# splinterhq/libsplinter

Hardware: AMD Instinct MI355X
Metric: KV set/get ops/sec + Nomic-768d embed vectors/sec at 1/2/4/8 MI355X (higher is better)
Workload: dtype bf16

## Files before the change

libsplinter_amd/csrc/hip/gemm_bf16.hip:

```cpp
#include <hip/hip_runtime.h>
#include <cstdint>
#include <cstdlib>
#include <map>
#include <mutex>
#include <type_traits>

#include "glds_asm.hpp"
#include "nomic_api.h"

namespace {

typedef __bf16 bf16x8 __attribute__((ext_vector_type(8)));
typedef float f32x4 __attribute__((ext_vector_type(4)));
typedef __attribute__((address_space(3))) void lds_void;
typedef const __attribute__((address_space(1))) void gbl_void;

constexpr int BM = 128, BN = 128, BK = 64;
constexpr int kThreads = 256;
constexpr int kTileBytes = BM * BK * 2;
constexpr int kEpiStride = BN + 4;
constexpr int kLdsBytes = (BM * kEpiStride * 4 > 4 * kTileBytes) ? BM * kEpiStride * 4 : 4 * kTileBytes;

__device__ __forceinline__ float bf2f(uint16_t h) { return __uint_as_float((uint32_t)h << 16); }
typedef __bf16 bf16x2_t __attribute__((ext_vector_type(2)));
// ... 39 lines not shown
  const uint16_t* res;
  long ldr;
  const float* rope;
  const int32_t* pos;
  int rope_cols;
  long M;
  int gn;
  const float2* pin;
  int np;
  float eps;
  const float* c1;
  const float* c2;
  const uint16_t* lng;
  const uint16_t* lnb;
  float2* part;
};

constexpr bool is_fold(int m) { return m == NOMIC_EPI_ROPE_FOLD || m == NOMIC_EPI_SWIGLU_FOLD; }
constexpr bool is_stats(int m) { return m == NOMIC_EPI_RES_STATS || m == NOMIC_EPI_RES_LN_STATS; }
constexpr bool is_rope(int m) { return m == NOMIC_EPI_ROPE || m == NOMIC_EPI_ROPE_FOLD; }
constexpr bool is_swiglu(int m) { return m == NOMIC_EPI_SWIGLU || m == NOMIC_EPI_SWIGLU_FOLD; }
constexpr bool is_rowstore(int m) { return m == NOMIC_EPI_STORE || m == NOMIC_EPI_RESIDUAL || is_stats(m); }
constexpr bool needs_rowstats(int m) { return is_fold(m) || m == NOMIC_EPI_RES_LN_STATS; }

__device__ __forceinline__ float fold(float acc, float2 st, float c1, float c2) {
  return st.y * (acc - st.x * c1) + c2;
}

template <int CTRL>
__device__ __forceinline__ float dpp_add(float v) {
// ... 256 lines not shown
    for (int it = 0; it < (BM * BN / 4) / kThreads; ++it) {
      const int q = tid + it * kThreads;
      const int row = q >> 5, c4 = (q & 31) * 4;
      const long gm = m0 + row;
      if (gm >= ep.M) continue;
      *(float4*)(outf + gm * ep.ldo + n0 + c4) = *(const float4*)&E[row * kEpiStride + c4];
    }
  }
}

constexpr int kThreads2 = 512;
constexpr int kHalfBytes = 128 * BK * 2;
constexpr int kBufBytes = 4 * kHalfBytes;
constexpr int kEpi2Stride = 256 + 4;
constexpr int kLds2Bytes = (128 * kEpi2Stride * 4 > 2 * kBufBytes) ? 128 * kEpi2Stride * 4 : 2 * kBufBytes;

__device__ __forceinline__ void wait_vm(int n) {
  switch (n) {
    case 26: asm volatile("s_waitcnt vmcnt(26)" ::: "memory"); break;
    case 20: asm volatile("s_waitcnt vmcnt(20)" ::: "memory"); break;
    case 18: asm volatile("s_waitcnt vmcnt(18)" ::: "memory"); break;
    case 10: asm volatile("s_waitcnt vmcnt(10)" ::: "memory"); break;
    case 8: asm volatile("s_waitcnt vmcnt(8)" ::: "memory"); break;
    case 6: asm volatile("s_waitcnt vmcnt(6)" ::: "memory"); break;
    case 4: asm volatile("s_waitcnt vmcnt(4)" ::: "memory"); break;
    case 2: asm volatile("s_waitcnt vmcnt(2)" ::: "memory"); break;
    default: asm volatile("s_waitcnt vmcnt(0)" ::: "memory"); break;
  }
}

// ... 8 lines not shown
  o.x = pk2(v[0], v[1]);
  o.y = pk2(v[2], v[3]);
  o.z = pk2(v[4], v[5]);
  o.w = pk2(v[6], v[7]);
  return o;
}

template <int MODE, int ILV = 0, int EPI = 0, int PP = 0>
__global__ __launch_bounds__(kThreads2, 1) void k_gemm256(const uint16_t* __restrict__ A, long lda,
                                                          const uint16_t* __restrict__ W, long ldw, int K,
                                                          int mtiles, int ntiles, EpiArgs ep) {
  extern __shared__ __attribute__((aligned(16))) char smem[];
  const int tid = threadIdx.x, lane = tid & 63, wave = tid >> 6;
  const int wr = wave >> 2, wn = wave & 3;
  int mt, nt;
  remap_tile(blockIdx.x, mtiles * ntiles, ntiles, ep.gn, mt, nt);
  const long m0 = (long)mt * 256, n0 = (long)nt * 256;

  const int srow = lane >> 3, schunk = ((lane & 7) ^ srow) * 8;
  uint32_t offA[2][2], offB[2][2];
#pragma unroll
  for (int h = 0; h < 2; ++h)
#pragma unroll
    for (int i = 0; i < 2; ++i) {
      const int r = h * 128 + (i * 8 + wave) * 8 + srow;
      const long gr = (m0 + r < ep.M) ? m0 + r : ep.M - 1;
      offA[h][i] = (uint32_t)(gr * lda + schunk);
      offB[h][i] = (uint32_t)((n0 + r) * ldw + schunk);
    }
  auto stage_one = [&](int which, int t, int buf, int i) {
    const uint16_t* base = (which < 2 ? A : W) + (long)t * BK;
    char* dst = smem + buf * kBufBytes + which * kHalfBytes;
// ... 11 lines not shown
  const int frow = (lane & 15) * 128;
  const int fsw0 = ((0 * 4 + (lane >> 4)) ^ (lane & 7)) << 4;
  const int fsw1 = ((1 * 4 + (lane >> 4)) ^ (lane & 7)) << 4;

  f32x4 acc[2][2][4][2];
#pragma unroll
  for (int a = 0; a < 2; ++a)
#pragma unroll
    for (int b = 0; b < 2; ++b)
#pragma unroll
      for (int i = 0; i < 4; ++i)
#pragma unroll
        for (int j = 0; j < 2; ++j) acc[a][b][i][j] = f32x4{0.f, 0.f, 0.f, 0.f};

  const int nk = K / BK;
  stage(0, 0, 0); stage(2, 0, 0); stage(3, 0, 0); stage(1, 0, 0);
  if (nk > 1) { stage(0, 1, 1); stage(2, 1, 1); stage(3, 1, 1); }

  bf16x8 af[4][2], b0[2][2], b1[2][2];
  auto mma_phase = [&](f32x4 (&ac)[4][2], bf16x8 (&bf)[2][2], int which, int st, int sbuf, bool go) {
    if (ILV == 0 && go) stage(which, st, sbuf);
    __builtin_amdgcn_s_setprio(1);
#pragma unroll
    for (int kk = 0; kk < 2; ++kk)
#pragma unroll
      for (int i = 0; i < 4; ++i) {
        if constexpr (ILV > 0) {
          if (go && kk * 4 + i == ILV) stage_one(which, st, sbuf, 0);
          if (go && kk * 4 + i == ILV + 4) stage_one(which, st, sbuf, 1);
        }
#pragma unroll
        for (int j = 0; j < 2; ++j)
          ac[i][j] = __builtin_amdgcn_mfma_f32_16x16x32_bf16(af[i][kk], bf[j][kk], ac[i][j], 0, 0, 0);
        if constexpr (ILV > 0) __builtin_amdgcn_sched_barrier(0);
// ... 186 lines not shown
    for (int j = 0; j < 2; ++j) {
      b1[j][0] = *(const bf16x8*)(hB1 + (wn * 32 + j * 16) * 128 + frow + fsw0);
      b1[j][1] = *(const bf16x8*)(hB1 + (wn * 32 + j * 16) * 128 + frow + fsw1);
    }
    mma_phase(acc[0][1], b1, 0, t + 2, buf, n2);
    wait_vm(n2 ? 10 : (n1 ? 8 : 0));
    raw_barrier();
#pragma unroll
    for (int i = 0; i < 4; ++i) {
      af[i][0] = *(const bf16x8*)(hA1 + (wr * 64 + i * 16) * 128 + frow + fsw0);
      af[i][1] = *(const bf16x8*)(hA1 + (wr * 64 + i * 16) * 128 + frow + fsw1);
    }
    mma_phase(acc[1][0], b0, 2, t + 2, buf, n2);
    mma_phase(acc[1][1], b1, 3, t + 2, buf, n2);
  }
  asm volatile("s_waitcnt vmcnt(0)" ::: "memory");

  if constexpr (MODE == NOMIC_EPI_SWIGLU && EPI == 1) {
    constexpr int kS = 128 + 8;
    uint16_t* E16 = (uint16_t*)smem;
    const int fq = lane >> 4, fr = lane & 15;
    const bool odd = fr & 1;
    __syncthreads();
#pragma unroll
    for (int qm = 0; qm < 2; ++qm)
#pragma unroll
      for (int qn = 0; qn < 2; ++qn)
#pragma unroll
        for (int i = 0; i < 4; ++i) {
          uint32_t b[4];
// ... 10 lines not shown
        }
    __syncthreads();
#pragma unroll
    for (int it = 0; it < (256 * 16) / kThreads2; ++it) {
      const int q = tid + it * kThreads2;
      const int row = q >> 4, c = q & 15;
      const long gm = m0 + row;
      if (gm >= ep.M) continue;
      *(uint4*)(ep.out + gm * ep.ldo + (long)nt * 128 + c * 8) = *(const uint4*)(E16 + row * kS + c * 8);
    }
    return;
  }

  float* E = (float*)smem;
  const int fq = lane >> 4, fr = lane & 15;
#pragma unroll
  for (int qm = 0; qm < 2; ++qm) {
    __syncthreads();
#pragma unroll
    for (int qn = 0; qn < 2; ++qn)
#pragma unroll
      for (int i = 0; i < 4; ++i)
#pragma unroll
        for (int j = 0; j < 2; ++j)
#pragma unroll
          for (int r = 0; r < 4; ++r)
            E[(wr * 64 + i * 16 + fq * 4 + r) * kEpi2Stride + qn * 128 + wn * 32 + j * 16 + fr] = acc[qm][qn][i][j][r];
    __syncthreads();
    const long mh = m0 + qm * 128;
    if constexpr (MODE == NOMIC_EPI_STORE || MODE == NOMIC_EPI_RESIDUAL) {
#pragma unroll
      for (int it = 0; it < (128 * 256 / 8) / kThreads2; ++it) {
        const int q = tid + it * kThreads2;
        const int row = q >> 5, c8 = (q & 31) * 8;
        const long gm = mh + row;
        if (gm >= ep.M) continue;
        const float4 v0 = *(const float4*)&E[row * kEpi2Stride + c8];
        const float4 v1 = *(const float4*)&E[row * kEpi2Stride + c8 + 4];
        float v[8] = {v0.x, v0.y, v0.z, v0.w, v1.x, v1.y, v1.z, v1.w};
        if constexpr (MODE == NOMIC_EPI_RESIDUAL) {
          const uint4 rr = *(const uint4*)(ep.res + gm * ep.ldr + n0 + c8);
          const uint32_t rw[4] = {rr.x, rr.y, rr.z, rr.w};
#pragma unroll
          for (int e = 0; e < 4; ++e) {
// ... 55 lines not shown
      for (int it = 0; it < (128 * 256 / 4) / kThreads2; ++it) {
        const int q = tid + it * kThreads2;
        const int row = q >> 6, c4 = (q & 63) * 4;
        const long gm = mh + row;
        if (gm >= ep.M) continue;
        *(float4*)(outf + gm * ep.ldo + n0 + c4) = *(const float4*)&E[row * kEpi2Stride + c4];
      }
    }
  }
}

}

namespace {

int g_num_cus = 256;

template <typename F>
void allow_lds(F* f, int bytes) {
  (void)hipFuncSetAttribute((const void*)f, hipFuncAttributeMaxDynamicSharedMemorySize, bytes);
}

int g_variant = -1;
int gemm_variant() {
  if (g_variant < 0) {
    const char* e = getenv("NOMIC_GEMM");
    const int v = e ? atoi(e) : 0;
    g_variant = v == 128 || v == 256 ? v : 0;
  }
  return g_variant;
}
// ... 13 lines not shown
template <int MODE>
int launch(const uint16_t* A, long lda, const uint16_t* W, long ldw, long M, int N, int K, EpiArgs ep,
           hipStream_t s) {
  if (K % BK || N % BN || M <= 0) return (int)hipErrorInvalidValue;
  const long mpad = (M + 255) / 256 * 256;
  const bool fits = N % 256 == 0 && mpad * lda < (1L << 31) && (long)N * ldw < (1L << 31);
  const int var = gemm_variant();
  constexpr bool k256_ok = MODE <= NOMIC_EPI_F32;
  const long tiles256 = fits ? (mpad / 256) * (N / 256) : 0;
  static const long min_tiles = [] {
    const char* e = getenv("NOMIC_GEMM256_MIN_TILES");
    return e && atol(e) > 0 ? atol(e) : 1024L;
  }();
  if (k256_ok && fits && (var == 256 || (var == 0 && tiles256 >= min_tiles))) {
    static bool attr = [] {
      allow_lds(k_gemm256<MODE, 0, 0, 2>, kLds2Bytes);
      return true;
    }();
    (void)attr;
    const int mtiles = (int)(mpad / 256), ntiles = N / 256;
    ep.gn = band_width(ntiles, 4);
    if constexpr (k256_ok)
      hipLaunchKernelGGL((k_gemm256<MODE, 0, 0, 2>), dim3(mtiles * ntiles), dim3(kThreads2), kLds2Bytes, s, A, lda, W,
                         ldw, K, mtiles, ntiles, ep);
    return (int)hipGetLastError();
  }
  const int mtiles = (int)((M + BM - 1) / BM), ntiles = N / BN;
  ep.gn = band_width(ntiles, 8);
  constexpr int lds = kLdsBytes + (needs_rowstats(MODE) ? BM * 8 : 0);
  hipLaunchKernelGGL(k_gemm_nt<MODE>, dim3(mtiles * ntiles), dim3(kThreads), lds, s, A, lda, W, ldw, K, mtiles, ntiles,
                     ep);
  return (int)hipGetLastError();
}

}

extern "C" int nomic_gemm_set_variant(int variant) {
  const int prev = gemm_variant();
  g_variant = variant == 128 || variant == 256 ? variant : 0;
  return prev;
}

extern "C" int nomic_gemm_ln(int mode, const void* A, long lda, const void* W, long ldw, long M, int N, int K,
                             void* out, long ldo, const void* res, long ldr, const float* rope, const int32_t* pos,
                             int rope_cols, const float* part_in, int nparts, float eps, const float* c1,
                             const float* c2, const void* ln_g, const void* ln_b, float* part, hipStream_t s) {
  EpiArgs ep{(uint16_t*)out, ldo, (const uint16_t*)res, ldr, rope, pos, rope_cols, M, 1, (const float2*)part_in,
             nparts, eps, c1, c2, (const uint16_t*)ln_g, (const uint16_t*)ln_b, (float2*)part};
  if ((needs_rowstats(mode) && (!part_in || nparts < 1 || nparts > 8)) || (is_fold(mode) && (!c1 || !c2)) ||
      (is_stats(mode) && (!part || !res || N % BN)) || (mode == NOMIC_EPI_RES_LN_STATS && (!ln_g || !ln_b)) ||
      (mode == NOMIC_EPI_RESIDUAL && !res) || (is_rope(mode) && (!rope || !pos)))
    return (int)hipErrorInvalidValue;
  const auto* a = (const uint16_t*)A;
  const auto* w = (const uint16_t*)W;
  switch (mode) {
// ... 46 lines not shown
```

libsplinter_amd/csrc/hip/gemm_rln.hip:

```cpp
#include <hip/hip_runtime.h>
#include <cstdint>
#include <cstdlib>

#include "glds_asm.hpp"
#include "nomic_api.h"

namespace {

typedef __bf16 bf16x8 __attribute__((ext_vector_type(8)));
typedef __bf16 bf16x2_t __attribute__((ext_vector_type(2)));
typedef float f32x4 __attribute__((ext_vector_type(4)));
typedef __attribute__((address_space(3))) void lds_void;
typedef const __attribute__((address_space(1))) void gbl_void;

constexpr int kBM = 128;
constexpr int kN = 768;
constexpr int kBK = 32;
constexpr int kWN = kN / 4;
constexpr int kNT = kWN / 16;
constexpr int kThreads = 512;
constexpr int kRowBytes = kBK * 2;
constexpr int kABytes = kBM * kRowBytes;
constexpr int kWBytes = kN * kRowBytes;
constexpr int kGldsW = kWBytes / 1024 / 8;
constexpr int kHalfRows = 64;
constexpr int kOutRowBytes = kN * 2;
constexpr int kRowPitch = kOutRowBytes + 16;
constexpr int kHalfBytes = kHalfRows * kRowPitch;
constexpr int kEpiLds = kHalfBytes + 2 * 4 * kHalfRows * 4;

template <int PIPE> struct Pipe;
template <> struct Pipe<1> { static constexpr int NW = 2, NA = 4; };
template <> struct Pipe<2> { static constexpr int NW = 3, NA = 2; };
template <> struct Pipe<3> { static constexpr int NW = 2, NA = 2; };
template <> struct Pipe<4> { static constexpr int NW = 2, NA = 6; };
template <int PIPE>
constexpr int lds_bytes() {
  return Pipe<PIPE>::NW * kWBytes + Pipe<PIPE>::NA * kABytes > kEpiLds
             ? Pipe<PIPE>::NW * kWBytes + Pipe<PIPE>::NA * kABytes
             : kEpiLds;
}

__device__ __forceinline__ float bf2f(uint32_t h16) { return __uint_as_float(h16 << 16); }
__device__ __forceinline__ uint32_t pk2(float a, float b) {
// ... 4 lines not shown
__device__ __forceinline__ void raw_barrier() {
  asm volatile("" ::: "memory");
  __builtin_amdgcn_s_barrier();
  asm volatile("" ::: "memory");
}

__device__ __forceinline__ void wait_vm(int n) {
  switch (n) {
    case 12: asm volatile("s_waitcnt vmcnt(12)" ::: "memory"); break;
    case 6: asm volatile("s_waitcnt vmcnt(6)" ::: "memory"); break;
    case 2: asm volatile("s_waitcnt vmcnt(2)" ::: "memory"); break;
    case 1: asm volatile("s_waitcnt vmcnt(1)" ::: "memory"); break;
    default: asm volatile("s_waitcnt vmcnt(0)" ::: "memory"); break;
  }
}

__device__ __forceinline__ int swz(int r, int c) { return c ^ ((r >> 1) & 3); }

template <int PIPE, int EPI, int WM, int ILV = 0, int PF = 1, bool AS = false, bool ROT = false>
__global__ __launch_bounds__(256 * WM, 1) void k_gemm_rln(const uint16_t* __restrict__ A, long lda,
                                                          const uint16_t* __restrict__ W, long ldw, int K, long M,
                                                          const uint16_t* res, long ldr,
                                                          const uint16_t* __restrict__ gamma,
                                                          const uint16_t* __restrict__ beta, float eps,
                                                          uint16_t* out, long ldo) {
  constexpr int NW = Pipe<PIPE>::NW, NA = Pipe<PIPE>::NA;
  constexpr int LW = NW - 1, LA = NA - 1;
  constexpr int kABase = NW * kWBytes;
  constexpr int kWaves = 4 * WM, kNThreads = 64 * kWaves;
  constexpr int RW = kBM / WM, MT = RW / 16;
  constexpr int GA = 8 / kWaves, GW = 48 / kWaves;
  static_assert(EPI == 0 || WM == 2, "the LDS-staged epilogue splits the tile by wave rows");
  static_assert(EPI != 3 || MT * kNT == 48, "EPI 3 spreads 48 accumulator tiles over 24 stages");
  extern __shared__ __attribute__((aligned(16))) char smem[];
  const int tid = threadIdx.x, lane = tid & 63, wave = tid >> 6;
  const int wr = WM == 2 ? wave >> 2 : 0, wn = wave & 3;
  const long m0 = (long)blockIdx.x * kBM;

  const int drow = lane >> 2, dpc = lane & 3;
  uint32_t offA[GA];
#pragma unroll
  for (int i = 0; i < GA; ++i) {
    const int r = (wave + kWaves * i) * 16 + drow;
    const long gr = (m0 + r < M) ? m0 + r : M - 1;
    offA[i] = (uint32_t)(gr * lda + swz(r, dpc) * 8);
  }
  uint32_t offW[GW];
#pragma unroll
// ... 86 lines not shown
  auto res_load = [&](int u, uint2& d) {
    const int i = u / kNT, j = u % kNT;
    const long m = rmb + 16 * i < M ? rmb + 16 * i : M - 1;
    d = *(const uint2*)(res + m * ldr + wn * kWN + j * 16 + rcq);
  };
  auto res_add = [&](int u, const uint2& rr) {
    const int i = u / kNT, j = u % kNT;
    acc[i][j][0] += bf2f(rr.x & 0xffff);
    acc[i][j][1] += bf2f(rr.x >> 16);
    acc[i][j][2] += bf2f(rr.y & 0xffff);
    acc[i][j][3] += bf2f(rr.y >> 16);
  };
  for (int t = 0; t < nk; ++t) {
    wait_vm(younger(t));
    raw_barrier();
    if (EPI == 3 && t < 24) {
#pragma unroll
      for (int k = 0; k < 24; ++k) {
        if (t == k) {
          if (k > 0) {
            res_add(2 * (k - 1), rq[0]);
            res_add(2 * (k - 1) + 1, rq[1]);
          }
          res_load(2 * k, rq[0]);
          res_load(2 * k + 1, rq[1]);
        }
      }
    }
    if (ILV == 0) issue(t);
    const char* bw = smem + (t % NW) * kWBytes;
    const char* ba = smem + (t % NA) * kABytes;
// ... 27 lines not shown
      }
      __builtin_amdgcn_sched_barrier(0);
      w0 = x0;
      w1 = x1;
      if (PF == 2) {
        x0 = y0;
        x1 = y1;
      }
    }
    __builtin_amdgcn_s_setprio(0);
    if (ILV > 0) {
#pragma unroll
      for (int u = (kNT / 2) * ILV; u < kOps; ++u) issue_op(t, u);
    }
  }
  if constexpr (EPI == 3) {
    res_add(46, rq[0]);
    res_add(47, rq[1]);
  }
  asm volatile("s_waitcnt vmcnt(0)" ::: "memory");
  raw_barrier();

  const int rl = lane & 15, cq = (lane >> 4) * 4;
  if constexpr (EPI != 1) {
    float* red = (float*)smem;
    const long mb = m0 + wr * RW + rl;
    float s[MT] = {};
#pragma unroll
    for (int j = 0; j < kNT; ++j) {
      const int n = wn * kWN + j * 16 + cq;
#pragma unroll
      for (int i = 0; i < MT; ++i) {
        if constexpr (EPI == 0) {
          const long m = mb + 16 * i < M ? mb + 16 * i : M - 1;
          const uint2 rr = *(const uint2*)(res + m * ldr + n);
          acc[i][j][0] += bf2f(rr.x & 0xffff);
          acc[i][j][1] += bf2f(rr.x >> 16);
          acc[i][j][2] += bf2f(rr.y & 0xffff);
          acc[i][j][3] += bf2f(rr.y >> 16);
        }
        (void)n;
        s[i] += (acc[i][j][0] + acc[i][j][1]) + (acc[i][j][2] + acc[i][j][3]);
      }
    }
#pragma unroll
    for (int i = 0; i < MT; ++i) {
      s[i] += __shfl_xor(s[i], 16);
      s[i] += __shfl_xor(s[i], 32);
    }
    if (lane < 16) {
#pragma unroll
      for (int i = 0; i < MT; ++i) red[wn * kBM + wr * RW + i * 16 + rl] = s[i];
    }
    __syncthreads();
    float mean[MT];
#pragma unroll
    for (int i = 0; i < MT; ++i) {
      const int r = wr * RW + i * 16 + rl;
      mean[i] = (red[r] + red[kBM + r] + red[2 * kBM + r] + red[3 * kBM + r]) * (1.f / kN);
// ... 14 lines not shown
      s[i] += __shfl_xor(s[i], 32);
    }
    __syncthreads();
    if (lane < 16) {
#pragma unroll
      for (int i = 0; i < MT; ++i) red[wn * kBM + wr * RW + i * 16 + rl] = s[i];
    }
    __syncthreads();
    float rstd[MT];
#pragma unroll
    for (int i = 0; i < MT; ++i) {
      const int r = wr * RW + i * 16 + rl;
      const float var = (red[r] + red[kBM + r] + red[2 * kBM + r] + red[3 * kBM + r]) * (1.f / kN);
      rstd[i] = rsqrtf(var + eps);
    }
#pragma unroll
    for (int j = 0; j < kNT; ++j) {
      const int n = wn * kWN + j * 16 + cq;
      const uint2 gg = *(const uint2*)(gamma + n), bb = *(const uint2*)(beta + n);
      const float g[4] = {bf2f(gg.x & 0xffff), bf2f(gg.x >> 16), bf2f(gg.y & 0xffff), bf2f(gg.y >> 16)};
      const float be[4] = {bf2f(bb.x & 0xffff), bf2f(bb.x >> 16), bf2f(bb.y & 0xffff), bf2f(bb.y >> 16)};
#pragma unroll
      for (int i = 0; i < MT; ++i) {
        const long m = mb + 16 * i;
        float o[4];
#pragma unroll
        for (int e = 0; e < 4; ++e) o[e] = (acc[i][j][e] - mean[i]) * rstd[i] * g[e] + be[e];
        if (m < M) *(uint2*)(out + m * ldo + n) = make_uint2(pk2(o[0], o[1]), pk2(o[2], o[3]));
      }
    }
  } else {
    char* R = smem;
    float* red1 = (float*)(smem + kHalfBytes);
    float* red2 = red1 + 4 * kHalfRows;
    const int ebase = rl * kRowPitch + (wn * kWN + cq) * 2;
#pragma unroll 1
    for (int h = 0; h < 2; ++h) {
      const long mh = m0 + h * kHalfRows;
#pragma unroll 1
      for (int u = 0; u < kHalfRows / 8; ++u) {
        const int row = wave * 8 + u;
        const long gr = mh + row < M ? mh + row : M - 1;
        const uint16_t* src = res + gr * ldr + lane * 8;
        __builtin_amdgcn_global_load_lds((gbl_void*)src, (lds_void*)(R + row * kRowPitch), 16, 0, 0);
        if (lane < 32)
          __builtin_amdgcn_global_load_lds((gbl_void*)(src + 512), (lds_void*)(R + row * kRowPitch + 1024), 16, 0, 0);
      }
      asm volatile("s_waitcnt vmcnt(0)" ::: "memory");
      __syncthreads();
      const bool mine = wr == h;
      float mean[4], rstd[4];
      if (mine) {
        float sm[4] = {0.f, 0.f, 0.f, 0.f};
#pragma unroll
        for (int j = 0; j < kNT; ++j) {
#pragma unroll
          for (int i = 0; i < 4; ++i) {
            const uint2 rr = *(const uint2*)(R + ebase + i * 16 * kRowPitch + j * 32);
            acc[i][j][0] += bf2f(rr.x & 0xffff);
            acc[i][j][1] += bf2f(rr.x >> 16);
            acc[i][j][2] += bf2f(rr.y & 0xffff);
            acc[i][j][3] += bf2f(rr.y >> 16);
            sm[i] += (acc[i][j][0] + acc[i][j][1]) + (acc[i][j][2] + acc[i][j][3]);
          }
        }
#pragma unroll
        for (int i = 0; i < 4; ++i) {
          sm[i] += __shfl_xor(sm[i], 16);
          sm[i] += __shfl_xor(sm[i], 32);
          if (lane < 16) red1[wn * kHalfRows + i * 16 + rl] = sm[i];
        }
      }
      __syncthreads();
      if (mine) {
        float sq[4] = {0.f, 0.f, 0.f, 0.f};
#pragma unroll
        for (int i = 0; i < 4; ++i) {
          const int r = i * 16 + rl;
          mean[i] = (red1[r] + red1[kHalfRows + r] + red1[2 * kHalfRows + r] + red1[3 * kHalfRows + r]) * (1.f / kN);
        }
#pragma unroll
        for (int j = 0; j < kNT; ++j)
#pragma unroll
          for (int i = 0; i < 4; ++i)
#pragma unroll
            for (int e = 0; e < 4; ++e) {
              const float d = acc[i][j][e] - mean[i];
              sq[i] += d * d;
            }
#pragma unroll
        for (int i = 0; i < 4; ++i) {
          sq[i] += __shfl_xor(sq[i], 16);
          sq[i] += __shfl_xor(sq[i], 32);
          if (lane < 16) red2[wn * kHalfRows + i * 16 + rl] = sq[i];
        }
      }
      __syncthreads();
      if (mine) {
#pragma unroll
        for (int i = 0; i < 4; ++i) {
          const int r = i * 16 + rl;
          const float var = (red2[r] + red2[kHalfRows + r] + red2[2 * kHalfRows + r] + red2[3 * kHalfRows + r]) *
                            (1.f / kN);
          rstd[i] = rsqrtf(var + eps);
        }
#pragma unroll
        for (int j = 0; j < kNT; ++j) {
          const int n = wn * kWN + j * 16 + cq;
          const uint2 gg = *(const uint2*)(gamma + n), bb = *(const uint2*)(beta + n);
          const float g[4] = {bf2f(gg.x & 0xffff), bf2f(gg.x >> 16), bf2f(gg.y & 0xffff), bf2f(gg.y >> 16)};
          const float be[4] = {bf2f(bb.x & 0xffff), bf2f(bb.x >> 16), bf2f(bb.y & 0xffff), bf2f(bb.y >> 16)};
#pragma unroll
          for (int i = 0; i < 4; ++i) {
            float o[4];
#pragma unroll
            for (int e = 0; e < 4; ++e) o[e] = (acc[i][j][e] - mean[i]) * rstd[i] * g[e] + be[e];
            *(uint2*)(R + ebase + i * 16 * kRowPitch + j * 32) = make_uint2(pk2(o[0], o[1]), pk2(o[2], o[3]));
          }
        }
      }
      __syncthreads();
#pragma unroll 2
      for (int u = 0; u < kHalfRows * 96 / kThreads; ++u) {
        const int L = u * kThreads + tid;
        const int row = L / 96, pc = L - row * 96;
        const uint4 v = *(const uint4*)(R + row * kRowPitch + pc * 16);
        if (mh + row < M) *(uint4*)(out + (mh + row) * ldo + pc * 8) = v;
      }
      __syncthreads();
    }
  }
}

int g_rln_variant = -1;
int rln_pick(int v) { return v == 232 ? 232 : 222; }
int rln_variant() {
  if (g_rln_variant < 0) {
    const char* e = getenv("NOMIC_RLN");
    g_rln_variant = rln_pick(e && *e ? atoi(e) : 222);
  }
  return g_rln_variant;
}

template <int PIPE, int EPI, int WM = 2, int ILV = 0, int PF = 1, bool AS = false, bool ROT = false>
void launch_rln(unsigned blocks, hipStream_t s, const uint16_t* A, long lda, const uint16_t* W, long ldw, int K, long M,
                const uint16_t* res, long ldr, const uint16_t* gamma, const uint16_t* beta, float eps, uint16_t* out,
                long ldo) {
  static bool attr = [] {
    (void)hipFuncSetAttribute((const void*)k_gemm_rln<PIPE, EPI, WM, ILV, PF, AS, ROT>, hipFuncAttributeMaxDynamicSharedMemorySize,
                              lds_bytes<PIPE>());
    return true;
  }();
  (void)attr;
  hipLaunchKernelGGL((k_gemm_rln<PIPE, EPI, WM, ILV, PF, AS, ROT>), dim3(blocks), dim3(256 * WM), lds_bytes<PIPE>(), s, A, lda, W, ldw, K,
// ... 6 lines not shown
                                 const void* res, long ldr, const void* gamma, const void* beta, float eps, void* out,
                                 long ldo, hipStream_t s) {
  if (N != kN || K < kBK || K % kBK || M <= 0 || !A || !W || !res || !gamma || !beta || !out)
    return (int)hipErrorInvalidValue;
  if (lda % 8 || ldw % 8 || ldr % 4 || ldo % 4 || lda < K || ldw < K || ldr < N || ldo < N)
    return (int)hipErrorInvalidValue;
  if ((M - 1) * lda + K >= (1L << 32) || (long)kN * ldw >= (1L << 32)) return (int)hipErrorInvalidValue;
  static_assert(lds_bytes<2>() <= 160 * 1024, "LDS budget");
  const unsigned blocks = (unsigned)((M + kBM - 1) / kBM);
  const auto* a = (const uint16_t*)A;
  const auto* w = (const uint16_t*)W;
  const auto* r = (const uint16_t*)res;
  const auto* g = (const uint16_t*)gamma;
  const auto* b = (const uint16_t*)beta;
  auto* o = (uint16_t*)out;
  if (rln_variant() == 232 && K / kBK >= 24 && K <= 768) launch_rln<2, 3, 2, 2>(blocks, s, a, lda, w, ldw, K, M, r, ldr, g, b, eps, o, ldo);
  else launch_rln<2, 0, 2, 2>(blocks, s, a, lda, w, ldw, K, M, r, ldr, g, b, eps, o, ldo);
  return (int)hipGetLastError();
}

extern "C" int nomic_gemm_res_ln_set_variant(int variant) {
  const int prev = rln_variant();
  g_rln_variant = rln_pick(variant);
  return prev;
}
```

libsplinter_amd/csrc/include/nomic_api.h:

```cpp
#ifndef SPLINTER_NOMIC_API_H
#define SPLINTER_NOMIC_API_H
#include <stdint.h>
#include "arena_api.h"

#ifdef __cplusplus
extern "C" {
#endif

#define NOMIC_EPI_STORE    0
#define NOMIC_EPI_RESIDUAL 1
#define NOMIC_EPI_SWIGLU   2
#define NOMIC_EPI_ROPE     3
#define NOMIC_EPI_F32      4
#define NOMIC_EPI_ROPE_FOLD    5
#define NOMIC_EPI_SWIGLU_FOLD  6
#define NOMIC_EPI_RES_STATS    7
#define NOMIC_EPI_RES_LN_STATS 8

int nomic_gemm(int mode, const void *A, long lda, const void *W, long ldw, long M, int N, int K,
               void *out, long ldo, const void *res, long ldr, const float *rope, const int32_t *pos,
               int rope_cols, hipStream_t stream);
int nomic_gemm_ln(int mode, const void *A, long lda, const void *W, long ldw, long M, int N, int K, void *out,
                  long ldo, const void *res, long ldr, const float *rope, const int32_t *pos, int rope_cols,
                  const float *part_in, int nparts, float eps, const float *c1, const float *c2,
                  const void *ln_g, const void *ln_b, float *part, hipStream_t stream);
int nomic_row_stats(const float *part, int nparts, long M, float eps, float *st, hipStream_t stream);
int nomic_gemm_set_variant(int variant);

int nomic_embed_ln(const int32_t *ids, long T, const void *tok_emb, const void *type_row,
                   const void *gamma, const void *beta, float eps, void *out, hipStream_t stream);
int nomic_layernorm(const void *x, long T, const void *gamma, const void *beta, float eps, void *out,
                    hipStream_t stream);
int nomic_attention_set_variant(int variant);
int nomic_attention(const void *qkv, void *out, const int32_t *cu_seqlens, const int32_t *qblocks,
                    int nqb, int heads, float scale, hipStream_t stream);
int nomic_mean_pool(const void *x, const int32_t *cu_seqlens, int B, float *pooled, int normalize,
                    spl_arena_t arena, const int64_t *slots, const uint64_t *hashes, int32_t *status,
                    hipStream_t stream);
int nomic_dequant(int ggml_type, const void *src, long nelems, void *dst_bf16, hipStream_t stream);

#ifdef __cplusplus
}
// ... 3 lines not shown
```

libsplinter_amd/models/nomic.py:

```python
from __future__ import annotations

import ctypes
import math
import os
from dataclasses import dataclass
from typing import Dict, List, Optional, Sequence, Tuple

import numpy as np
import torch

from .. import _native as N
from ..utils.tracing import trace_range
from .gguf import DEVICE_DEQUANT, GGUFFile, GGUFWriter, dequant_host

EPI_STORE, EPI_RESIDUAL, EPI_SWIGLU, EPI_ROPE, EPI_F32 = 0, 1, 2, 3, 4
EPI_ROPE_FOLD, EPI_SWIGLU_FOLD, EPI_RES_STATS, EPI_RES_LN_STATS = 5, 6, 7, 8


@dataclass
class NomicConfig:
    vocab: int = 30528
    d: int = 768
    layers: int = 12
    heads: int = 12
# ... 24 lines not shown
        P, c_long, c_int, c_float = ctypes.c_void_p, ctypes.c_long, ctypes.c_int, ctypes.c_float
        L.nomic_gemm.argtypes = [c_int, P, c_long, P, c_long, c_long, c_int, c_int, P, c_long, P, c_long, P, P, c_int, P]
        L.nomic_gemm.restype = c_int
        L.nomic_gemm_ln.argtypes = [c_int, P, c_long, P, c_long, c_long, c_int, c_int, P, c_long, P, c_long, P, P,
                                    c_int, P, c_int, c_float, P, P, P, P, P, P]
        L.nomic_gemm_ln.restype = c_int
        L.nomic_gemm_res_ln.argtypes = [P, c_long, P, c_long, c_long, c_int, c_int, P, c_long, P, P, c_float, P,
                                        c_long, P]
        L.nomic_gemm_res_ln.restype = c_int
        L.nomic_gemm_res_ln_set_variant.argtypes = [c_int]
        L.nomic_gemm_res_ln_set_variant.restype = c_int
        L.nomic_row_stats.argtypes = [P, c_int, c_long, c_float, P, P]
        L.nomic_row_stats.restype = c_int
        L.nomic_gemm_set_variant.argtypes = [c_int]
        L.nomic_gemm_set_variant.restype = c_int
        L.nomic_attention_set_variant.argtypes = [c_int]
        L.nomic_attention_set_variant.restype = c_int
        L.nomic_embed_ln.argtypes = [P, c_long, P, P, P, P, c_float, P, P]
        L.nomic_embed_ln.restype = c_int
        L.nomic_layernorm.argtypes = [P, c_long, P, P, c_float, P, P]
        L.nomic_layernorm.restype = c_int
        L.nomic_attention.argtypes = [P, P, P, P, c_int, c_int, c_float, P]
        L.nomic_attention.restype = c_int
        L.nomic_mean_pool.argtypes = [P, P, c_int, P, c_int, N.Arena, P, P, P, P]
        L.nomic_mean_pool.restype = c_int
        L.nomic_dequant.argtypes = [c_int, P, c_long, P, P]
        L.nomic_dequant.restype = c_int
        L._nomic_declared = True
    return L

# ... 457 lines not shown
```

Baseline: 1.339 billion.

## Split tail-wave GEMM tiles into half-M blocks and add register-resident residual-LN epilogue

The 256x256 GEMM kernel now launches extra blocks for the last partial wave. Those tiles are split into two 128-row halves, each run by its own block with a three-slot pipeline, so CUs are not left idle at the tail. The CU count is now read from the device instead of being hard-coded. The residual+LayerNorm GEMM gains a new default epilogue (variant 242) that does 16-byte residual loads and stores with ds_swizzle lane exchange instead of 8-byte accesses, and the old LDS-staged epilogue is removed. The costs are extra LDS per block when splitting, a second mainloop path in the kernel, and possible tuning sensitivity.

```diff
diff --git a/libsplinter_amd/csrc/hip/gemm_bf16.hip b/libsplinter_amd/csrc/hip/gemm_bf16.hip
--- a/libsplinter_amd/csrc/hip/gemm_bf16.hip
+++ b/libsplinter_amd/csrc/hip/gemm_bf16.hip
@@ -77,6 +77,7 @@
   const uint16_t* lng;
   const uint16_t* lnb;
   float2* part;
+  int nsplit;
 };
 
 constexpr bool is_fold(int m) { return m == NOMIC_EPI_ROPE_FOLD || m == NOMIC_EPI_SWIGLU_FOLD; }
@@ -363,6 +364,8 @@
 constexpr int kBufBytes = 4 * kHalfBytes;
 constexpr int kEpi2Stride = 256 + 4;
 constexpr int kLds2Bytes = (128 * kEpi2Stride * 4 > 2 * kBufBytes) ? 128 * kEpi2Stride * 4 : 2 * kBufBytes;
+constexpr int kLds2SplitBytes = 9 * kHalfBytes;
+static_assert(kLds2SplitBytes >= kLds2Bytes && kLds2SplitBytes <= 160 * 1024, "LDS budget");
 
 __device__ __forceinline__ void wait_vm(int n) {
   switch (n) {
@@ -401,8 +404,23 @@
   const int tid = threadIdx.x, lane = tid & 63, wave = tid >> 6;
   const int wr = wave >> 2, wn = wave & 3;
   int mt, nt;
-  remap_tile(blockIdx.x, mtiles * ntiles, ntiles, ep.gn, mt, nt);
+  int bid = blockIdx.x, qh = -1;
+  {
+    const int nw = mtiles * ntiles - ep.nsplit;
+    if (bid >= nw) {
+      const int h = bid - nw, full = (ep.nsplit >> 3) << 4;
+      if (h < full) {
+        bid = nw + ((h >> 4) << 3) + (h & 7);
+        qh = (h >> 3) & 1;
+      } else {
+        bid = nw + (full >> 1) + ((h - full) >> 1);
+        qh = (h - full) & 1;
+      }
+    }
+  }
+  remap_tile(bid, mtiles * ntiles, ntiles, ep.gn, mt, nt);
   const long m0 = (long)mt * 256, n0 = (long)nt * 256;
+  if (qh >= 0 && m0 + qh * 128 >= ep.M) return;
 
   const int srow = lane >> 3, schunk = ((lane & 7) ^ srow) * 8;
   uint32_t offA[2][2], offB[2][2];
@@ -444,10 +462,88 @@
         for (int j = 0; j < 2; ++j) acc[a][b][i][j] = f32x4{0.f, 0.f, 0.f, 0.f};
 
   const int nk = K / BK;
+  bf16x8 af[4][2], b0[2][2], b1[2][2];
+  if (qh >= 0) {
+    constexpr int kStage3 = 3 * kHalfBytes;
+    const uint32_t oA[2] = {qh ? offA[1][0] : offA[0][0], qh ? offA[1][1] : offA[0][1]};
+    auto hstage = [&](int which, int t, int slot) {
+      const uint16_t* base = (which == 0 ? A : W) + (long)t * BK;
+      char* dst = smem + slot * kStage3 + which * kHalfBytes;
+#pragma unroll
+      for (int i = 0; i < 2; ++i) {
+        const uint32_t off = which == 0 ? oA[i] : which == 1 ? offB[0][i] : offB[1][i];
+        if constexpr (PP == 2)
+          spl::glds16_asm(base + off, dst + (i * 8 + wave) * 1024);
+        else
+          __builtin_amdgcn_global_load_lds((gbl_void*)(base + off), (lds_void*)(dst + (i * 8 + wave) * 1024), 16, 0,
+                                           0);
+      }
+    };
+    auto rd = [](bf16x8& dst, const char* p) {
+      dst = *(const bf16x8*)p;
+      __builtin_amdgcn_sched_barrier(0);
+    };
+    auto mm = [&](f32x4 (&ac)[4][2], bf16x8 (&bf)[2][2], int kk) {
+#pragma unroll
+      for (int i = 0; i < 4; ++i)
+#pragma unroll
+        for (int j = 0; j < 2; ++j)
+          ac[i][j] = __builtin_amdgcn_mfma_f32_16x16x32_bf16(af[i][kk], bf[j][kk], ac[i][j], 0, 0, 0);
+      __builtin_amdgcn_sched_barrier(0);
+    };
+    hstage(0, 0, 0); hstage(1, 0, 0); hstage(2, 0, 0);
+    if (nk > 1) { hstage(0, 1, 1); hstage(1, 1, 1); hstage(2, 1, 1); }
+    int slot = 0, sslot = 2;
+    auto h_kt = [&](int t, auto n1c, auto n2c) {
+      constexpr bool n1 = decltype(n1c)::value, n2 = decltype(n2c)::value;
+      const char* hA = smem + slot * kStage3;
+      const char* pa = hA + (wr * 64) * 128 + frow;
+      const char* pb0 = hA + kHalfBytes + (wn * 32) * 128 + frow;
+      const char* pb1 = hA + 2 * kHalfBytes + (wn * 32) * 128 + frow;
+      wait_vm(n1 ? 6 : 0);
+      raw_barrier();
+      __builtin_amdgcn_sched_barrier(0);
+#pragma unroll
+      for (int kk = 0; kk < 2; ++kk) {
+        const int fs = kk ? fsw1 : fsw0;
+        rd(b0[0][kk], pb0 + fs);
+        rd(b0[1][kk], pb0 + 16 * 128 + fs);
+#pragma unroll
+        for (int i = 0; i < 4; ++i) rd(af[i][kk], pa + i * 16 * 128 + fs);
+      }
+      if constexpr (n2) hstage(0, t + 2, sslot);
+      __builtin_amdgcn_sched_barrier(0);
+      __builtin_amdgcn_s_setprio(1);
+      mm(acc[0][0], b0, 0);
+      mm(acc[0][0], b0, 1);
+      __builtin_amdgcn_s_setprio(0);
+#pragma unroll
+      for (int kk = 0; kk < 2; ++kk) {
+        const int fs = kk ? fsw1 : fsw0;
+        rd(b1[0][kk], pb1 + fs);
+        rd(b1[1][kk], pb1 + 16 * 128 + fs);
+      }
+      if constexpr (n2) hstage(1, t + 2, sslot);
+      __builtin_amdgcn_sched_barrier(0);
+      __builtin_amdgcn_s_setprio(1);
+      mm(acc[0][1], b1, 0);
+      __builtin_amdgcn_s_setprio(0);
+      if constexpr (n2) hstage(2, t + 2, sslot);
+      __builtin_amdgcn_sched_barrier(0);
+      __builtin_amdgcn_s_setprio(1);
+      mm(acc[0][1], b1, 1);
+      __builtin_amdgcn_s_setprio(0);
+      slot = slot == 2 ? 0 : slot + 1;
+      sslot = sslot == 2 ? 0 : sslot + 1;
+    };
+    int t = 0;
+    for (; t + 2 < nk; ++t) h_kt(t, std::true_type{}, std::true_type{});
+    if (t + 1 < nk) h_kt(t++, std::true_type{}, std::false_type{});
+    if (t < nk) h_kt(t, std::false_type{}, std::false_type{});
+  } else {
   stage(0, 0, 0); stage(2, 0, 0); stage(3, 0, 0); stage(1, 0, 0);
   if (nk > 1) { stage(0, 1, 1); stage(2, 1, 1); stage(3, 1, 1); }
 
-  bf16x8 af[4][2], b0[2][2], b1[2][2];
   auto mma_phase = [&](f32x4 (&ac)[4][2], bf16x8 (&bf)[2][2], int which, int st, int sbuf, bool go) {
     if (ILV == 0 && go) stage(which, st, sbuf);
     __builtin_amdgcn_s_setprio(1);
@@ -664,6 +760,7 @@
     mma_phase(acc[1][0], b0, 2, t + 2, buf, n2);
     mma_phase(acc[1][1], b1, 3, t + 2, buf, n2);
   }
+  }
   asm volatile("s_waitcnt vmcnt(0)" ::: "memory");
 
   if constexpr (MODE == NOMIC_EPI_SWIGLU && EPI == 1) {
@@ -704,8 +801,10 @@
 
   float* E = (float*)smem;
   const int fq = lane >> 4, fr = lane & 15;
+  const long mbase = m0 + (qh > 0 ? 128 : 0);
 #pragma unroll
   for (int qm = 0; qm < 2; ++qm) {
+    if (qm == 1 && qh >= 0) break;
     __syncthreads();
 #pragma unroll
     for (int qn = 0; qn < 2; ++qn)
@@ -717,7 +816,7 @@
           for (int r = 0; r < 4; ++r)
             E[(wr * 64 + i * 16 + fq * 4 + r) * kEpi2Stride + qn * 128 + wn * 32 + j * 16 + fr] = acc[qm][qn][i][j][r];
     __syncthreads();
-    const long mh = m0 + qm * 128;
+    const long mh = mbase + qm * 128;
     if constexpr (MODE == NOMIC_EPI_STORE || MODE == NOMIC_EPI_RESIDUAL) {
 #pragma unroll
       for (int it = 0; it < (128 * 256 / 8) / kThreads2; ++it) {
@@ -803,7 +902,30 @@
 
 namespace {
 
-int g_num_cus = 256;
+int g_num_cus = 0;
+int num_cus() {
+  if (g_num_cus <= 0) {
+    int dev = 0, n = 0;
+    if (hipGetDevice(&dev) != hipSuccess ||
+        hipDeviceGetAttribute(&n, hipDeviceAttributeMultiprocessorCount, dev) != hipSuccess || n <= 0)
+      n = 256;
+    g_num_cus = n;
+  }
+  return g_num_cus;
+}
+
+int g_tail_split = -1;
+int tail_split() {
+  if (g_tail_split < 0) {
+    const char* e = getenv("NOMIC_GEMM_TAIL_SPLIT");
+    g_tail_split = e && *e ? atoi(e) != 0 : 1;
+  }
+  return g_tail_split;
+}
+int split_tiles(long T) {
+  const int cus = num_cus(), R = (int)(T % cus);
+  return tail_split() && R > 0 && R <= cus / 2 ? R : 0;
+}
 
 template <typename F>
 void allow_lds(F* f, int bytes) {
@@ -847,15 +969,16 @@
   }();
   if (k256_ok && fits && (var == 256 || (var == 0 && tiles256 >= min_tiles))) {
     static bool attr = [] {
-      allow_lds(k_gemm256<MODE, 0, 0, 2>, kLds2Bytes);
+      allow_lds(k_gemm256<MODE, 0, 0, 2>, kLds2SplitBytes);
       return true;
     }();
     (void)attr;
     const int mtiles = (int)(mpad / 256), ntiles = N / 256;
     ep.gn = band_width(ntiles, 4);
+    ep.nsplit = split_tiles(tiles256);
     if constexpr (k256_ok)
-      hipLaunchKernelGGL((k_gemm256<MODE, 0, 0, 2>), dim3(mtiles * ntiles), dim3(kThreads2), kLds2Bytes, s, A, lda, W,
-                         ldw, K, mtiles, ntiles, ep);
+      hipLaunchKernelGGL((k_gemm256<MODE, 0, 0, 2>), dim3(mtiles * ntiles + ep.nsplit), dim3(kThreads2),
+                         ep.nsplit ? kLds2SplitBytes : kLds2Bytes, s, A, lda, W, ldw, K, mtiles, ntiles, ep);
     return (int)hipGetLastError();
   }
   const int mtiles = (int)((M + BM - 1) / BM), ntiles = N / BN;
@@ -872,6 +995,18 @@
   const int prev = gemm_variant();
   g_variant = variant == 128 || variant == 256 ? variant : 0;
   return prev;
+}
+
+extern "C" int nomic_gemm_set_tail_split(int on) {
+  const int prev = tail_split();
+  g_tail_split = on != 0;
+  return prev;
+}
+
+extern "C" long nomic_gemm256_grid(long M, int N) {
+  if (M <= 0 || N <= 0 || N % 256) return 0;
+  const long T = (M + 255) / 256 * (N / 256);
+  return T + split_tiles(T);
 }
 
 extern "C" int nomic_gemm_ln(int mode, const void* A, long lda, const void* W, long ldw, long M, int N, int K,
diff --git a/libsplinter_amd/csrc/hip/gemm_rln.hip b/libsplinter_amd/csrc/hip/gemm_rln.hip
--- a/libsplinter_amd/csrc/hip/gemm_rln.hip
+++ b/libsplinter_amd/csrc/hip/gemm_rln.hip
@@ -23,11 +23,7 @@
 constexpr int kABytes = kBM * kRowBytes;
 constexpr int kWBytes = kN * kRowBytes;
 constexpr int kGldsW = kWBytes / 1024 / 8;
-constexpr int kHalfRows = 64;
-constexpr int kOutRowBytes = kN * 2;
-constexpr int kRowPitch = kOutRowBytes + 16;
-constexpr int kHalfBytes = kHalfRows * kRowPitch;
-constexpr int kEpiLds = kHalfBytes + 2 * 4 * kHalfRows * 4;
+constexpr int kEpiLds = 4 * kBM * 4;
 
 template <int PIPE> struct Pipe;
 template <> struct Pipe<1> { static constexpr int NW = 2, NA = 4; };
@@ -62,6 +58,8 @@
     default: asm volatile("s_waitcnt vmcnt(0)" ::: "memory"); break;
   }
 }
+
+__device__ __forceinline__ uint32_t xor16(uint32_t v) { return (uint32_t)__builtin_amdgcn_ds_swizzle((int)v, 0x401F); }
 
 __device__ __forceinline__ int swz(int r, int c) { return c ^ ((r >> 1) & 3); }
 
@@ -78,8 +76,10 @@
   constexpr int kWaves = 4 * WM, kNThreads = 64 * kWaves;
   constexpr int RW = kBM / WM, MT = RW / 16;
   constexpr int GA = 8 / kWaves, GW = 48 / kWaves;
-  static_assert(EPI == 0 || WM == 2, "the LDS-staged epilogue splits the tile by wave rows");
-  static_assert(EPI != 3 || MT * kNT == 48, "EPI 3 spreads 48 accumulator tiles over 24 stages");
+  constexpr bool KRES = EPI == 3;
+  constexpr bool WIDE = EPI == 4;
+  static_assert(EPI == 0 || EPI == 2 || EPI == 3 || EPI == 4, "epilogue forms");
+  static_assert(!KRES || MT * kNT == 48, "EPI 3 spreads 48 accumulator tiles over 24 stages");
   extern __shared__ __attribute__((aligned(16))) char smem[];
   const int tid = threadIdx.x, lane = tid & 63, wave = tid >> 6;
   const int wr = WM == 2 ? wave >> 2 : 0, wn = wave & 3;
@@ -196,7 +196,7 @@
   for (int t = 0; t < nk; ++t) {
     wait_vm(younger(t));
     raw_barrier();
-    if (EPI == 3 && t < 24) {
+    if (KRES && t < 24) {
 #pragma unroll
       for (int k = 0; k < 24; ++k) {
         if (t == k) {
@@ -254,7 +254,7 @@
       for (int u = (kNT / 2) * ILV; u < kOps; ++u) issue_op(t, u);
     }
   }
-  if constexpr (EPI == 3) {
+  if constexpr (KRES) {
     res_add(46, rq[0]);
     res_add(47, rq[1]);
   }
@@ -262,10 +262,36 @@
   raw_barrier();
 
   const int rl = lane & 15, cq = (lane >> 4) * 4;
-  if constexpr (EPI != 1) {
+  {
     float* red = (float*)smem;
     const long mb = m0 + wr * RW + rl;
     float s[MT] = {};
+    const bool odd = (lane >> 4) & 1;
+    const int c8 = wn * kWN + (odd ? 16 : 0) + (lane >> 5) * 8;
+    (void)odd, (void)c8;
+    if constexpr (EPI == 4) {
+#pragma unroll
+      for (int p = 0; p < kNT / 2; ++p) {
+#pragma unroll
+        for (int i = 0; i < MT; ++i) {
+          const long m = mb + 16 * i < M ? mb + 16 * i : M - 1;
+          const uint4 rr = *(const uint4*)(res + m * ldr + c8 + 32 * p);
+          const uint32_t gx = xor16(odd ? rr.x : rr.z), gy = xor16(odd ? rr.y : rr.w);
+          const uint32_t r0[2] = {odd ? gx : rr.x, odd ? gy : rr.y};
+          const uint32_t r1[2] = {odd ? rr.z : gx, odd ? rr.w : gy};
+#pragma unroll
+          for (int h = 0; h < 2; ++h) {
+            const int j = 2 * p + h;
+            const uint32_t x = h ? r1[0] : r0[0], y = h ? r1[1] : r0[1];
+            acc[i][j][0] += bf2f(x & 0xffff);
+            acc[i][j][1] += bf2f(x >> 16);
+            acc[i][j][2] += bf2f(y & 0xffff);
+            acc[i][j][3] += bf2f(y >> 16);
+            s[i] += (acc[i][j][0] + acc[i][j][1]) + (acc[i][j][2] + acc[i][j][3]);
+          }
+        }
+      }
+    } else {
 #pragma unroll
     for (int j = 0; j < kNT; ++j) {
       const int n = wn * kWN + j * 16 + cq;
@@ -283,6 +309,7 @@
         s[i] += (acc[i][j][0] + acc[i][j][1]) + (acc[i][j][2] + acc[i][j][3]);
       }
     }
+    }
 #pragma unroll
     for (int i = 0; i < MT; ++i) {
       s[i] += __shfl_xor(s[i], 16);
@@ -327,6 +354,35 @@
       const float var = (red[r] + red[kBM + r] + red[2 * kBM + r] + red[3 * kBM + r]) * (1.f / kN);
       rstd[i] = rsqrtf(var + eps);
     }
+    if constexpr (WIDE) {
+#pragma unroll
+      for (int p = 0; p < kNT / 2; ++p) {
+        float g[2][4], be[2][4];
+#pragma unroll
+        for (int h = 0; h < 2; ++h) {
+          const int n = wn * kWN + (2 * p + h) * 16 + cq;
+          const uint2 gg = *(const uint2*)(gamma + n), bb = *(const uint2*)(beta + n);
+          g[h][0] = bf2f(gg.x & 0xffff), g[h][1] = bf2f(gg.x >> 16), g[h][2] = bf2f(gg.y & 0xffff), g[h][3] = bf2f(gg.y >> 16);
+          be[h][0] = bf2f(bb.x & 0xffff), be[h][1] = bf2f(bb.x >> 16), be[h][2] = bf2f(bb.y & 0xffff), be[h][3] = bf2f(bb.y >> 16);
+        }
+#pragma unroll
+        for (int i = 0; i < MT; ++i) {
+          const long m = mb + 16 * i;
+          uint32_t pk[2][2];
+#pragma unroll
+          for (int h = 0; h < 2; ++h) {
+            float o[4];
+#pragma unroll
+            for (int e = 0; e < 4; ++e) o[e] = (acc[i][2 * p + h][e] - mean[i]) * rstd[i] * g[h][e] + be[h][e];
+            pk[h][0] = pk2(o[0], o[1]);
+            pk[h][1] = pk2(o[2], o[3]);
+          }
+          const uint32_t gx = xor16(odd ? pk[0][0] : pk[1][0]), gy = xor16(odd ? pk[0][1] : pk[1][1]);
+          const uint4 v = odd ? make_uint4(gx, gy, pk[1][0], pk[1][1]) : make_uint4(pk[0][0], pk[0][1], gx, gy);
+          if (m < M) *(uint4*)(out + m * ldo + c8 + 32 * p) = v;
+        }
+      }
+    } else {
 #pragma unroll
     for (int j = 0; j < kNT; ++j) {
       const int n = wn * kWN + j * 16 + cq;
@@ -342,115 +398,16 @@
         if (m < M) *(uint2*)(out + m * ldo + n) = make_uint2(pk2(o[0], o[1]), pk2(o[2], o[3]));
       }
     }
-  } else {
-    char* R = smem;
-    float* red1 = (float*)(smem + kHalfBytes);
-    float* red2 = red1 + 4 * kHalfRows;
-    const int ebase = rl * kRowPitch + (wn * kWN + cq) * 2;
-#pragma unroll 1
-    for (int h = 0; h < 2; ++h) {
-      const long mh = m0 + h * kHalfRows;
-#pragma unroll 1
-      for (int u = 0; u < kHalfRows / 8; ++u) {
-        const int row = wave * 8 + u;
-        const long gr = mh + row < M ? mh + row : M - 1;
-        const uint16_t* src = res + gr * ldr + lane * 8;
-        __builtin_amdgcn_global_load_lds((gbl_void*)src, (lds_void*)(R + row * kRowPitch), 16, 0, 0);
-        if (lane < 32)
-          __builtin_amdgcn_global_load_lds((gbl_void*)(src + 512), (lds_void*)(R + row * kRowPitch + 1024), 16, 0, 0);
-      }
-      asm volatile("s_waitcnt vmcnt(0)" ::: "memory");
-      __syncthreads();
-      const bool mine = wr == h;
-      float mean[4], rstd[4];
-      if (mine) {
-        float sm[4] = {0.f, 0.f, 0.f, 0.f};
-#pragma unroll
-        for (int j = 0; j < kNT; ++j) {
-#pragma unroll
-          for (int i = 0; i < 4; ++i) {
-            const uint2 rr = *(const uint2*)(R + ebase + i * 16 * kRowPitch + j * 32);
-            acc[i][j][0] += bf2f(rr.x & 0xffff);
-            acc[i][j][1] += bf2f(rr.x >> 16);
-            acc[i][j][2] += bf2f(rr.y & 0xffff);
-            acc[i][j][3] += bf2f(rr.y >> 16);
-            sm[i] += (acc[i][j][0] + acc[i][j][1]) + (acc[i][j][2] + acc[i][j][3]);
-          }
-        }
-#pragma unroll
-        for (int i = 0; i < 4; ++i) {
-          sm[i] += __shfl_xor(sm[i], 16);
-          sm[i] += __shfl_xor(sm[i], 32);
-          if (lane < 16) red1[wn * kHalfRows + i * 16 + rl] = sm[i];
-        }
-      }
-      __syncthreads();
-      if (mine) {
-        float sq[4] = {0.f, 0.f, 0.f, 0.f};
-#pragma unroll
-        for (int i = 0; i < 4; ++i) {
-          const int r = i * 16 + rl;
-          mean[i] = (red1[r] + red1[kHalfRows + r] + red1[2 * kHalfRows + r] + red1[3 * kHalfRows + r]) * (1.f / kN);
-        }
-#pragma unroll
-        for (int j = 0; j < kNT; ++j)
-#pragma unroll
-          for (int i = 0; i < 4; ++i)
-#pragma unroll
-            for (int e = 0; e < 4; ++e) {
-              const float d = acc[i][j][e] - mean[i];
-              sq[i] += d * d;
-            }
-#pragma unroll
-        for (int i = 0; i < 4; ++i) {
-          sq[i] += __shfl_xor(sq[i], 16);
-          sq[i] += __shfl_xor(sq[i], 32);
-          if (lane < 16) red2[wn * kHalfRows + i * 16 + rl] = sq[i];
-        }
-      }
-      __syncthreads();
-      if (mine) {
-#pragma unroll
-        for (int i = 0; i < 4; ++i) {
-          const int r = i * 16 + rl;
-          const float var = (red2[r] + red2[kHalfRows + r] + red2[2 * kHalfRows + r] + red2[3 * kHalfRows + r]) *
-                            (1.f / kN);
-          rstd[i] = rsqrtf(var + eps);
-        }
-#pragma unroll
-        for (int j = 0; j < kNT; ++j) {
-          const int n = wn * kWN + j * 16 + cq;
-          const uint2 gg = *(const uint2*)(gamma + n), bb = *(const uint2*)(beta + n);
-          const float g[4] = {bf2f(gg.x & 0xffff), bf2f(gg.x >> 16), bf2f(gg.y & 0xffff), bf2f(gg.y >> 16)};
-          const float be[4] = {bf2f(bb.x & 0xffff), bf2f(bb.x >> 16), bf2f(bb.y & 0xffff), bf2f(bb.y >> 16)};
-#pragma unroll
-          for (int i = 0; i < 4; ++i) {
-            float o[4];
-#pragma unroll
-            for (int e = 0; e < 4; ++e) o[e] = (acc[i][j][e] - mean[i]) * rstd[i] * g[e] + be[e];
-            *(uint2*)(R + ebase + i * 16 * kRowPitch + j * 32) = make_uint2(pk2(o[0], o[1]), pk2(o[2], o[3]));
-          }
-        }
-      }
-      __syncthreads();
-#pragma unroll 2
-      for (int u = 0; u < kHalfRows * 96 / kThreads; ++u) {
-        const int L = u * kThreads + tid;
-        const int row = L / 96, pc = L - row * 96;
-        const uint4 v = *(const uint4*)(R + row * kRowPitch + pc * 16);
-        if (mh + row < M) *(uint4*)(out + (mh + row) * ldo + pc * 8) = v;
-      }
-      __syncthreads();
     }
   }
 }
 
 int g_rln_variant = -1;
-int rln_pick(int v) { return v == 232 ? 232 : 222; }
+int rln_pick(int v) { return v == 222 || v == 232 ? v : 242; }
 int rln_variant() {
   if (g_rln_variant < 0) {
     const char* e = getenv("NOMIC_RLN");
-    g_rln_variant = rln_pick(e && *e ? atoi(e) : 222);
+    g_rln_variant = rln_pick(e && *e ? atoi(e) : 242);
   }
   return g_rln_variant;
 }
@@ -487,7 +444,12 @@
   const auto* g = (const uint16_t*)gamma;
   const auto* b = (const uint16_t*)beta;
   auto* o = (uint16_t*)out;
-  if (rln_variant() == 232 && K / kBK >= 24 && K <= 768) launch_rln<2, 3, 2, 2>(blocks, s, a, lda, w, ldw, K, M, r, ldr, g, b, eps, o, ldo);
+  const bool wide_ok = ldr % 8 == 0 && ldo % 8 == 0 && ((uintptr_t)res | (uintptr_t)out) % 16 == 0;
+  int v = rln_variant();
+  if (v == 232 && !(K / kBK >= 24 && K <= 768)) v = 222;
+  if (v == 242 && !wide_ok) v = 222;
+  if (v == 232) launch_rln<2, 3, 2, 2>(blocks, s, a, lda, w, ldw, K, M, r, ldr, g, b, eps, o, ldo);
+  else if (v == 242) launch_rln<2, 4, 2, 2>(blocks, s, a, lda, w, ldw, K, M, r, ldr, g, b, eps, o, ldo);
   else launch_rln<2, 0, 2, 2>(blocks, s, a, lda, w, ldw, K, M, r, ldr, g, b, eps, o, ldo);
   return (int)hipGetLastError();
 }
diff --git a/libsplinter_amd/csrc/include/nomic_api.h b/libsplinter_amd/csrc/include/nomic_api.h
--- a/libsplinter_amd/csrc/include/nomic_api.h
+++ b/libsplinter_amd/csrc/include/nomic_api.h
@@ -26,6 +26,8 @@
                   const void *ln_g, const void *ln_b, float *part, hipStream_t stream);
 int nomic_row_stats(const float *part, int nparts, long M, float eps, float *st, hipStream_t stream);
 int nomic_gemm_set_variant(int variant);
+int nomic_gemm_set_tail_split(int on);
+long nomic_gemm256_grid(long M, int N);
 
 int nomic_embed_ln(const int32_t *ids, long T, const void *tok_emb, const void *type_row,
                    const void *gamma, const void *beta, float eps, void *out, hipStream_t stream);
diff --git a/libsplinter_amd/models/nomic.py b/libsplinter_amd/models/nomic.py
--- a/libsplinter_amd/models/nomic.py
+++ b/libsplinter_amd/models/nomic.py
@@ -62,6 +62,10 @@
         L.nomic_row_stats.restype = c_int
         L.nomic_gemm_set_variant.argtypes = [c_int]
         L.nomic_gemm_set_variant.restype = c_int
+        L.nomic_gemm_set_tail_split.argtypes = [c_int]
+        L.nomic_gemm_set_tail_split.restype = c_int
+        L.nomic_gemm256_grid.argtypes = [c_long, c_int]
+        L.nomic_gemm256_grid.restype = c_long
         L.nomic_attention_set_variant.argtypes = [c_int]
         L.nomic_attention_set_variant.restype = c_int
         L.nomic_embed_ln.argtypes = [P, c_long, P, P, P, P, c_float, P, P]
```

Measured after the change: 1.368 billion (median of 6 runs). 2.2% higher.
